# adolfogonzalez3/maddpg

Measured on AMD Instinct MI355X. Metric: env-steps/sec (end-to-end at the reference update cadence), simple_spread N=3, batch 1024, higher is better.
Workload: dtype fp32

## Files before the change

maddpg_amd/csrc/mdp_api.cpp:

```cpp
#include <hip/hip_runtime.h>

#include <algorithm>
#include <cmath>
#include <cstdio>
#include <cstdlib>
#include <cstring>
#include <string>
#include <dlfcn.h>
#include <rccl/rccl.h>

#include <map>
#include <vector>

#include "mdp_kernels.h"

namespace {

inline int64_t r4(int64_t n) { return (n + 3) & ~int64_t(3); }
inline int64_t a256(int64_t n) { return (n + 255) & ~int64_t(255); }

NDesc make_net(int64_t& off, int in, int H, int out) {
  NDesc d;
  d.off = (int)off;
  d.in = in;
// ... 247 lines not shown
  *pos = 624;
}

}

struct mdp_handle {
  mdp_config cfg;
  Layout L;
  int device = 0;
  hipStream_t stream = nullptr;
  bool own_stream = false;
  char* arena = nullptr;
  float *theta, *target, *m, *v, *grad, *replay, *beta, *slab_c, *slab_a, *eplog;
  float *pos, *vel, *ep_rew;
  float* env_comm = nullptr;
  int32_t *index, *goal, *ep_step;
  double *stats, *stat_c, *stat_a, *y;
  Ctl* ctl;
  int64_t len = 0, next = 0;
  uint32_t act_ctr = 0, reset_ctr = 0;
  bool env_lockstep = true;
  std::string err;
  bool ready = false;
  bool prof_on[MDP_K_COUNT] = {};
  std::vector<hipEvent_t> ev[MDP_K_COUNT];
  size_t ev_used[MDP_K_COUNT] = {};
  double prof_ms[MDP_K_COUNT] = {};
  int64_t prof_n[MDP_K_COUNT] = {};
  bool graphs = true;
  bool capturing = false;
  int eager_rounds = 0;
  bool general_grads = false;
  bool fused_apply = true;
  uint32_t* ra_ctr = nullptr;
  uint64_t* ra_part = nullptr;
  float* apre = nullptr;
  bool actor_pre = true;
  float* cpre = nullptr;
  bool critic_pre = true;
  float* apre_rows = nullptr;
  float* cpre_rows = nullptr;
  std::map<std::vector<int>, hipGraphExec_t> graph_exec;
  int eager_steps = 0;
  ncclComm_t comm = nullptr;
  int dp_world = 1;
  bool dp_graphs = false;
  int update_mode = 0;
  FusedApplyArgs* tp_list = nullptr;
  RaBatch tp_batch;
  RaBatch tp_reduce, tp_step;
  int ra_cap = 0, ra_batch_cap = 0;
  bool tp_fits[4] = {true, true, true, true};
  std::vector<FusedApplyArgs> tp_host[4];
  RaBatch tp_xchg;
  RaBatch tp_pair[3][MDP_MAX_AGENTS];
  bool tp_pair_fits[3][MDP_MAX_AGENTS] = {};
  FusedApplyArgs tp_pair_host[3][MDP_MAX_AGENTS][2];
  bool rollout_draw = true;
  bool draw_ahead = true;
  bool grad_pair = true;
  uint64_t* xbuf = nullptr;
  int x_world = 0, x_rank = 0;
  std::vector<void*> x_opened;
  XchgDesc* xd_dev = nullptr;
  uint32_t* x_probe = nullptr;
  uint32_t x_probe_ep = 0;
// ... 680 lines not shown
  if (h->x_probe) (void)hipFree(h->x_probe);
  if (h->xbuf) (void)hipFree(h->xbuf);
  h->xd_dev = nullptr;
  h->x_probe = nullptr;
  h->xbuf = nullptr;
  h->p2p = false;
  h->x_world = 0;
  h->x_rank = 0;
}

int launch_reduce(mdp_handle* h, const OptNet& o) {
  const ReduceArgs a = reduce_args(h, o);
  ProfScope p(h, MDP_K_REDUCE);
  HIPCHK(h, mdp_launch_reduce(a, h->stream));
  return 0;
}

int launch_apply(mdp_handle* h, const OptNet& o, float scale) {
  const ApplyArgs a = apply_args(h, o, scale);
  ProfScope p(h, MDP_K_APPLY);
  HIPCHK(h, mdp_launch_apply(a, h->stream));
  return 0;
}

int opt_step(mdp_handle* h, const OptNet& o, bool fused, float scale, int32_t* pf_out = nullptr, int pf_count = 0) {
  if (fused) {
    FusedApplyArgs f = fused_args(h, o, scale);
    if (pf_out && pf_count > 0) {
      f.pf_out = pf_out;
      f.pf_count = pf_count;
    }
    if (h->p2p && o.own) set_xchg(h, f);
    ProfScope p(h, MDP_K_REDUCE_APPLY);
    HIPCHK(h, mdp_launch_reduce_apply(f, h->stream));
    return 0;
  }
  const int rc = launch_reduce(h, o);
  if (rc) return rc;
  OptNet a = o;
  if (!o.own) a.bump_ctr = 0;
  return launch_apply(h, a, scale);
}

struct RcclApi {
  bool tried = false, ok = false;
  decltype(&ncclGetUniqueId) get_id = nullptr;
  decltype(&ncclCommInitRank) init_rank = nullptr;
  decltype(&ncclAllReduce) all_reduce = nullptr;
  decltype(&ncclCommDestroy) destroy = nullptr;
  decltype(&ncclGetErrorString) err = nullptr;
  decltype(&ncclCommCount) count = nullptr;
};
RcclApi& rccl() {
  static RcclApi r;
  if (!r.tried) {
    r.tried = true;
    const char* alt = getenv("MDP_RCCL_LIB");
    void* so = nullptr;
    if (alt && alt[0]) {
      so = dlopen(alt, RTLD_NOW | RTLD_LOCAL);
    } else {
      so = dlopen("librccl.so.1", RTLD_NOW | RTLD_LOCAL);
      if (!so) so = dlopen("/opt/rocm/lib/librccl.so.1", RTLD_NOW | RTLD_LOCAL);
    }
    if (so) {
      r.get_id = (decltype(r.get_id))dlsym(so, "ncclGetUniqueId");
      r.init_rank = (decltype(r.init_rank))dlsym(so, "ncclCommInitRank");
// ... 167 lines not shown

bool tp_ok(const mdp_handle* h) {
  if (!h->fused_apply) return false;
  for (int i = 0; i < h->cfg.n_agents; ++i)
    if (!reduce_apply_ok(h, i, 0) || !reduce_apply_ok(h, i, 1)) return false;
  return 2 * h->cfg.n_agents <= MDP_RA_BATCH_MAX;
}

FusedApplyArgs tp_args(mdp_handle* h, int agent, int net) {
  const int64_t nwg = h->L.nwg;
  OptNet o = opt_own(h, agent, net);
  o.slab += agent * nwg * o.slab_stride;
  o.slab_stat += agent * nwg * 8;
  o.y += (int64_t)agent * h->cfg.batch_size;
  o.polyak = 1;
  o.bump_ctr = (net == 0 && agent == 0) ? h->cfg.n_agents : 0;
  FusedApplyArgs f = fused_args(h, o);
  for (int t = 0; t < 7; ++t) f.ap.oblk[t] = 0;
  return f;
}

int tp_setup(mdp_handle* h) {
  if (h->tp_list) {
    (void)hipFree(h->tp_list);
    h->tp_list = nullptr;
  }
  const int n = h->cfg.n_agents;
  std::vector<FusedApplyArgs> list;
  RaBatch* rbs[4] = {&h->tp_batch, &h->tp_reduce, &h->tp_step, &h->tp_xchg};
  for (int ph = 0; ph < 4; ++ph) {
    RaBatch& rb = *rbs[ph];
    rb.count = 2 * n;
    rb.narrow = h->L.nwg <= 64 ? 1 : 0;
    rb.wg_start[0] = 0;
    for (int i = 0; i < n; ++i)
      for (int net = 1; net >= 0; --net) {
        FusedApplyArgs f = tp_args(h, i, net);
        f.phase = ph;
        if (ph == 2) f.ap.scale = 1.0f / (float)h->dp_world;
        if (ph == 3) {
          if (h->p2p) set_xchg(h, f);
          else f.phase = 0;
        }
        list.push_back(f);
        const int q = 2 * i + (1 - net);
        rb.wg_start[q + 1] = rb.wg_start[q] + mdp_ra_grid(f);
      }
  }
  for (int ph = 0; ph < 4; ++ph) {
    h->tp_host[ph].assign(list.begin() + 2 * n * ph, list.begin() + 2 * n * (ph + 1));
    h->tp_fits[ph] = ph == 1 || rbs[ph]->wg_start[2 * n] <= h->ra_batch_cap;
  }
  const int pair_phase[3] = {0, 1, 3};
  const size_t pair0 = list.size();
  for (int pp = 0; pp < 3; ++pp)
    for (int i = 0; i < n; ++i) {
      RaBatch& rb = h->tp_pair[pp][i];
      rb = RaBatch();
      rb.count = 2;
      rb.narrow = h->L.nwg <= 64 ? 1 : 0;
      for (int k = 0; k < 2; ++k) {
        const int net = 1 - k;
        FusedApplyArgs f = tp_args(h, i, net);
        f.ap.slab = net ? h->slab_c : h->slab_a;
        f.ap.polyak = 0;
        f.ap.bump_ctr = (net == 0 && i == n - 1) ? n : 0;
        f.phase = pair_phase[pp];
        if (pp == 2) {
          if (h->p2p) set_xchg(h, f);
          else f.phase = 0;
        }
        list.push_back(f);
        h->tp_pair_host[pp][i][k] = f;
        rb.wg_start[k + 1] = rb.wg_start[k] + mdp_ra_grid(f);
      }
      h->tp_pair_fits[pp][i] = pp == 1 || rb.wg_start[2] + 1 <= h->ra_batch_cap;
    }
  HIPCHK(h, hipMalloc((void**)&h->tp_list, sizeof(FusedApplyArgs) * list.size()));
  HIPCHK(h, hipMemcpy(h->tp_list, list.data(), sizeof(FusedApplyArgs) * list.size(), hipMemcpyHostToDevice));
  for (int ph = 0; ph < 4; ++ph) rbs[ph]->list = h->tp_list + (int64_t)ph * 2 * n;
  for (int pp = 0; pp < 3; ++pp)
    for (int i = 0; i < n; ++i) h->tp_pair[pp][i].list = h->tp_list + pair0 + (int64_t)(pp * n + i) * 2;
  return 0;
}

int dp_allreduce_all(mdp_handle* h);
int launch_tp_batch(mdp_handle* h, int ph);

int tp_grads_fast(mdp_handle* h, const int32_t* idx, const float* u_tgt, const float* u_act, int32_t* pf_out) {
  const int n = h->cfg.n_agents;
  const int64_t nwg = h->L.nwg;
  int lds_c = 0;
  for (int i = 0; i < n; ++i) lds_c = std::max(lds_c, lds_critic_r_bytes(h->L.topo, i));
  {
    CriticArgs a;
    a.apre = nullptr;
    a.apre_rows = nullptr;
    a.u_act = nullptr;
    a.cpre = nullptr;
    a.cpre_rows = nullptr;
    a.cpre_prev = -1;
    a.pf_ctl = h->ctl;
    a.pf_out = pf_out;
    a.pf_count = pf_out ? n * h->cfg.batch_size : 0;
    a.topo = h->L.topo;
    a.agent = 0;
    a.B = h->cfg.batch_size;
    a.theta = h->theta;
// ... 38 lines not shown
    a.slab = h->slab_a;
    a.slab_stride = h->L.slab_a;
    a.slab_stat = h->stat_a;
    a.multi = n;
    a.slab_agent_stride = nwg * h->L.slab_a;
    ProfScope p(h, MDP_K_ACTOR_GRAD);
    HIPCHK(h, mdp_launch_actor_grad_r(a, lds_actor_r_bytes(h->L.topo), h->stream));
  }
  return 0;
}

int launch_tp_pair(mdp_handle* h, int pp, int i, int32_t* piece) {
  const int B = h->cfg.batch_size;
  const int kind = pp == 1 ? MDP_K_REDUCE : MDP_K_REDUCE_APPLY;
  if (h->tp_pair_fits[pp][i]) {
    RaBatch rb = h->tp_pair[pp][i];
    if (piece) {
      rb.pf_out = piece;
      rb.pf_count = B;
      rb.pf_ctl = h->ctl;
    }
    ProfScope p(h, kind);
    HIPCHK(h, mdp_launch_reduce_apply_batch(rb, h->stream));
    return 0;
  }
  for (int k = 0; k < 2; ++k) {
    FusedApplyArgs f = h->tp_pair_host[pp][i][k];
    if (piece) {
      f.pf_out = piece + (k ? (B + 1) / 2 : 0);
      f.pf_count = k ? B - (B + 1) / 2 : (B + 1) / 2;
      f.pf_ctl = h->ctl;
    }
    ProfScope p(h, kind);
    HIPCHK(h, mdp_launch_reduce_apply(f, h->stream));
  }
  return 0;
}

int tp_round_general(mdp_handle* h, const int32_t* idx, const float* u_tgt, const float* u_act, int32_t* draw_out) {
  const int n = h->cfg.n_agents;
  const int64_t B = h->cfg.batch_size;
  const int pp = h->comm ? 1 : h->p2p ? 2 : 0;
  int rc;
  for (int i = 0; i < n; ++i) {
    const int32_t* ix = idx + i * B;
    const float* ut = u_tgt ? u_tgt + i * n * B * MDP_ACT_DIM : nullptr;
    const float* ua = u_act ? u_act + i * B * MDP_ACT_DIM : nullptr;
    if (h->grad_pair) {
      GradPairArgs g;
      g.c = critic_args(h, i, ix, ut, true, -1, nullptr, true);
      g.x = actor_args(h, i, ix, ua, true, false, -1, nullptr, true);
      const int lds = std::max(lds_critic_bytes(h->L.topo, g.c.group), lds_actor_bytes(h->L.topo));
      if (lds > MDP_LDS_BUDGET) return fail(h, "gradient pair does not fit in LDS");
      ProfScope p(h, MDP_K_CRITIC_GRAD);
      HIPCHK(h, mdp_launch_grad_pair(g, h->L.topo.H, lds, h->stream));
    } else {
      if ((rc = do_critic_grad(h, i, ix, ut, nullptr, true, false, nullptr, -1, 0, true))) return rc;
      if ((rc = do_actor_grad(h, i, ix, ua, true, false, -1, nullptr, true))) return rc;
    }
    if ((rc = launch_tp_pair(h, pp, i, draw_out ? draw_out + i * B : nullptr))) return rc;
  }
  if (h->comm) {
    if ((rc = dp_allreduce_all(h))) return rc;
    ProfScope p(h, MDP_K_APPLY, h->tp_fits[2]);
    return launch_tp_batch(h, 2);
  }
  float pa, pb;
  polyak_coef(h, &pa, &pb);
  HIPCHK(h, mdp_launch_polyak(h->target, h->theta, h->L.PT, pa, pb, h->ctl, h->stream));
  return 0;
}

int launch_tp_batch(mdp_handle* h, int ph) {
  const RaBatch* rbs[4] = {&h->tp_batch, &h->tp_reduce, &h->tp_step, &h->tp_xchg};
  if (h->tp_fits[ph]) {
    HIPCHK(h, mdp_launch_reduce_apply_batch(*rbs[ph], h->stream));
    return 0;
  }
  for (const FusedApplyArgs& f : h->tp_host[ph]) HIPCHK(h, mdp_launch_reduce_apply(f, h->stream));
  return 0;
}

int do_round_tp(mdp_handle* h, const int32_t* idx, const float* u_tgt, const float* u_act, int32_t* pf_out,
                int32_t* draw_out = nullptr) {
  if (!tp_fast(h)) return tp_round_general(h, idx, u_tgt, u_act, draw_out ? draw_out : pf_out);
  const int rc = tp_grads_fast(h, idx, u_tgt, u_act, pf_out);
  if (rc) return rc;
  if (h->p2p) {
    ProfScope p(h, MDP_K_REDUCE_APPLY, h->tp_fits[3]);
    return launch_tp_batch(h, 3);
  }
  if (h->comm) {
    {
      ProfScope p(h, MDP_K_REDUCE, h->tp_fits[1]);
      const int rc = launch_tp_batch(h, 1);
      if (rc) return rc;
    }
    const int rc = dp_allreduce_all(h);
    if (rc) return rc;
    ProfScope p(h, MDP_K_APPLY, h->tp_fits[2]);
    return launch_tp_batch(h, 2);
  }
  ProfScope p(h, MDP_K_REDUCE_APPLY, h->tp_fits[0]);
  return launch_tp_batch(h, 0);
}

int set_ring(mdp_handle* h, int64_t len, int64_t next) {
  h->len = len;
  h->next = next;
  HIPCHK(h, mdp_launch_set_ring(h->ctl, len, next, h->stream));
  return 0;
}
// ... 205 lines not shown
}

int mdp_ra_plan(const mdp_config* cfg, int32_t cus, int32_t per_cu, int32_t* out) {
  Layout L;
  std::string err;
  if (!build_layout(cfg, L, err) || cus < 0 || per_cu < 0) return -1;
  int fallback = 0;
  for (int i = 0; i < cfg->n_agents; ++i)
    for (int net = 0; net < 2; ++net) {
      const int g = mdp_ra_grid_of(L.topo, i, net);
      const bool ok = mdp_ra_fits(L.topo, i, net, cus * per_cu);
      if (out) out[2 * i + net] = ok ? g : -g;
      fallback += ok ? 0 : 1;
    }
  return fallback;
}

int mdp_create(const mdp_config* cfg, void* arena_dev, int64_t arena_bytes, void* hip_stream, mdp_handle** out) {
  if (!out) return -1;
  *out = nullptr;
  mdp_handle* h = new mdp_handle();
  std::string err;
  if (!build_layout(cfg, h->L, err)) {
    h->err = err;
    *out = h;
    return -1;
  }
  h->cfg = *cfg;
  {
    const char* g = getenv("MDP_GENERAL_GRADS");
    h->general_grads = g && g[0] == '1';
    const char* u = getenv("MDP_UNFUSED_APPLY");
    h->fused_apply = !(u && u[0] == '1');
    const char* rd = getenv("MDP_ROLLOUT_DRAW");
    h->rollout_draw = !(rd && rd[0] == '0');
    const char* da = getenv("MDP_DRAW_AHEAD");
    h->draw_ahead = !(da && da[0] == '0');
    const char* gp = getenv("MDP_GRAD_PAIR");
    h->grad_pair = !(gp && gp[0] == '0');
    const char* ap = getenv("MDP_ACTOR_PRE");
    h->actor_pre = !(ap && ap[0] == '0');
    const char* cp = getenv("MDP_CRITIC_PRE");
    h->critic_pre = !(cp && cp[0] == '0');
  }
  if (!arena_dev || arena_bytes < h->L.total) {
    h->err = "arena missing or too small";
    *out = h;
    return -1;
  }
  *out = h;
  HIPCHK(h, hipGetDevice(&h->device));
  if (need_dev(h, arena_dev, h->L.total, "mdp_create", "arena_dev", false)) return -1;
  {
    int cus = 0, per = 0, per_b = 0;
    HIPCHK(h, hipDeviceGetAttribute(&cus, hipDeviceAttributeMultiprocessorCount, h->device));
    HIPCHK(h, mdp_ra_occupancy(&per));
    HIPCHK(h, mdp_ra_batch_occupancy(&per_b));
    h->ra_cap = cus * per;
    h->ra_batch_cap = cus * per_b;
    int scratch = 0;
    HIPCHK(h, mdp_spin_kernels_scratch(&scratch));
    if (scratch > 0) h->ra_cap = h->ra_batch_cap = 0;
  }
  if (hip_stream) {
    h->stream = (hipStream_t)hip_stream;
  } else {
// ... 1905 lines not shown
```

maddpg_amd/csrc/mdp_apply_fused.hip:

```cpp
#include "mdp_device.h"
#include "mdp_kernels.h"
#include "mdp_mt.h"

namespace {
typedef double f64x4 __attribute__((ext_vector_type(4)));
constexpr uint32_t kSpinLimit = 1u << 22;

__device__ __forceinline__ void st_agent(double* p, double v) {
  __hip_atomic_store(p, v, __ATOMIC_RELAXED, __HIP_MEMORY_SCOPE_AGENT);
}
__device__ __forceinline__ double ld_agent(const double* p) {
  return __hip_atomic_load(const_cast<double*>(p), __ATOMIC_RELAXED, __HIP_MEMORY_SCOPE_AGENT);
}
__device__ __forceinline__ void st_agent64(uint64_t* p, uint64_t v) {
  __hip_atomic_store(p, v, __ATOMIC_RELAXED, __HIP_MEMORY_SCOPE_AGENT);
}
__device__ __forceinline__ uint64_t ld_agent64(const uint64_t* p) {
  return __hip_atomic_load(const_cast<uint64_t*>(p), __ATOMIC_RELAXED, __HIP_MEMORY_SCOPE_AGENT);
}

constexpr uint64_t kXchgTimeoutTicks = 30ull * 100000000ull;

__device__ __forceinline__ uint64_t ll_word(float v, uint32_t ep) {
  return ((uint64_t)ep << 32) | (uint64_t)__float_as_uint(v);
// ... 97 lines not shown
  hipLaunchKernelGGL(k_xchg_probe, dim3(nchunk), dim3(64), 0, s, xd, ep, bad, fault);
  return hipGetLastError();
}

#ifdef MDP_STAMPS
__device__ unsigned long long g_ra_ph[2][1024][8];
#define MDP_RA_PH(k)                                                                                     \
  do {                                                                                                   \
    if (threadIdx.x == 0 && b < 1024) g_ra_ph[a.stats_mode == 1 ? 0 : 1][b][k] = __builtin_amdgcn_s_memrealtime(); \
  } while (0)
extern "C" int mdp_debug_ra_phases(unsigned long long* out) {
  return hipMemcpyFromSymbol(out, HIP_SYMBOL(g_ra_ph), sizeof(g_ra_ph)) == hipSuccess ? 0 : -1;
}
extern "C" int mdp_debug_ra_phases_reset() {
  void* p = nullptr;
  if (hipGetSymbolAddress(&p, HIP_SYMBOL(g_ra_ph)) != hipSuccess) return -1;
  return hipMemset(p, 0, sizeof(unsigned long long) * 2 * 1024 * 8) == hipSuccess && hipDeviceSynchronize() == hipSuccess
             ? 0 : -1;
}
#else
#define MDP_RA_PH(k) \
  do {               \
  } while (0)
#endif

template <int LO, int N>
__device__ __forceinline__ f32x4 red_tree(const f32x4 (*red)[64], int col) {
  if constexpr (N == 1)
    return red[LO][col];
  else
    return red_tree<LO, N / 2>(red, col) + red_tree<LO + N / 2, N / 2>(red, col);
}

template <int G>
__device__ __forceinline__ void reduce_apply_body(const FusedApplyArgs& f, const int b, const uint32_t nb) {
  const ApplyArgs& a = f.ap;
  __shared__ f32x4 red[G][64];
  __shared__ f32x4 gl[64];
  __shared__ float step_l[4];
  const int tid = threadIdx.x, lane = tid & 63;
  MDP_STAMP(30);
  MDP_RA_PH(0);
  if (f.phase == 1 && b >= f.rblk[6]) return;
  if (b < f.rblk[6]) {
    int t = 0;
    while (b >= f.rblk[t + 1]) ++t;
    const TDesc td = a.net.t[t];
    const int n = td.rows * td.cols;
    const int nch = f.rblk[t + 1] - f.rblk[t];
    const int c = b - f.rblk[t];
    const int col = tid & 63, grp = tid >> 6;
    const int p0 = c * MDP_RA_CHUNK + 4 * col;
    const bool act = p0 < n;
    const int64_t i0 = td.off + p0;
    const int pq = c * MDP_RA_CHUNK + 64 * grp + lane;
    const bool aact = grp < 4 && pq < n;
    const int64_t iq = td.off + pq;
    float m1 = 0.f, v1 = 0.f, th1 = 0.f, tg1 = 0.f;
    const float b1p = a.beta[0], b2p = a.beta[1];
    const uint32_t ep_raw = f.phase == 3 ? f.xstep[0] : 0u;
    const uint32_t nep = f.sync_ctr[7 * 32] + 1u;
    uint32_t fault0 = 0u;
    if (grp == 0) fault0 = __hip_atomic_load(&a.ctl->fault, __ATOMIC_RELAXED, __HIP_MEMORY_SCOPE_AGENT);
    bool faulted = false;
    if (aact && f.phase != 1) {
      m1 = a.m[iq];
      v1 = a.v[iq];
      th1 = a.theta[iq];
      if (a.polyak) tg1 = a.target[iq];
    }
    f32x4 s = {0.f, 0.f, 0.f, 0.f};
    if constexpr (G == 16) {
      if (f.phase == 2) {
        if (grp == 0 && act) s = ld4(a.grad + i0);
      } else if (act) {
        const float* base = a.slab + (td.off - a.net.off) + p0;
        f32x4 v[16];
// ... 229 lines not shown
    const uint32_t prev = __hip_atomic_fetch_add(f.done_ctr, 1u, __ATOMIC_RELAXED, __HIP_MEMORY_SCOPE_AGENT);
    if (prev % nb == nb - 1) {
      if (__hip_atomic_load(&a.ctl->fault, __ATOMIC_RELAXED, __HIP_MEMORY_SCOPE_AGENT) == 0u) {
        const float p1 = a.beta[0], p2 = a.beta[1];
        a.beta[2] = p1;
        a.beta[3] = p2;
        a.beta[0] = p1 * a.b1;
        a.beta[1] = p2 * a.b2;
      }
      if (a.bump_ctr) a.ctl->upd_ctr += (uint32_t)a.bump_ctr;
      if (f.phase == 3) f.xstep[0] += 1u;
      f.sync_ctr[7 * 32] += 1u;
    }
  }
}

#ifdef MDP_STAMPS
__device__ unsigned long long g_ra_t0[1024], g_ra_t1[1024];
#define MDP_RA_WG(arr)                                                                 \
  do {                                                                                 \
    if (threadIdx.x == 0 && blockIdx.x < 1024) arr[blockIdx.x] = __builtin_amdgcn_s_memrealtime(); \
  } while (0)
extern "C" int mdp_debug_ra_wg(unsigned long long* t0, unsigned long long* t1, int n) {
  if (hipMemcpyFromSymbol(t0, HIP_SYMBOL(g_ra_t0), sizeof(unsigned long long) * n) != hipSuccess) return -1;
  return hipMemcpyFromSymbol(t1, HIP_SYMBOL(g_ra_t1), sizeof(unsigned long long) * n) == hipSuccess ? 0 : -1;
}
#else
#define MDP_RA_WG(arr) \
  do {                 \
  } while (0)
#endif


template <int NT>
__global__ __launch_bounds__(NT) void k_reduce_apply(FusedApplyArgs f) {
  MDP_RA_WG(g_ra_t0);
  MDP_TL(f.ap.ctl, f.ap.polyak ? 3 : 1, blockIdx.x == gridDim.x - 1 && f.pf_count > 0 ? 3 : 0);
  MDP_KARG_TOUCH("s"(f.pf_count), "s"(f.xstep), "s"(f.ap.blk[0]), "s"(f.ap.target), "s"(f.ap.clip), "s"(f.ap.stats_mode),
                 "s"(f.ap.ctl), "s"(gridDim.x), "s"(f.ap.net.t[0].off), "s"(f.ap.net.t[4].cols), "s"(f.ap.other.t[2].off),
                 "s"(f.ap.other.in));
  if (f.pf_count > 0 && blockIdx.x == gridDim.x - 1) {
    make_index_block<NT>(f.pf_ctl, f.pf_count, f.pf_out);
    __syncthreads();
    MDP_RA_WG(g_ra_t1);
    return;
  }
  reduce_apply_body<NT / 64>(f, blockIdx.x, gridDim.x - (f.pf_count > 0 ? 1 : 0));
#ifdef MDP_STAMPS
  __syncthreads();
  MDP_RA_WG(g_ra_t1);
#endif
}

template <int NT>
__global__ __launch_bounds__(NT) void k_reduce_apply_batch(RaBatch rb) {
  if (rb.pf_count > 0 && blockIdx.x == gridDim.x - 1) {
    make_index_block<NT>(rb.pf_ctl, rb.pf_count, rb.pf_out);
    return;
  }
  int q = 0;
  while (q + 1 < rb.count && (int)blockIdx.x >= rb.wg_start[q + 1]) ++q;
  const int b = blockIdx.x - rb.wg_start[q];
  reduce_apply_body<NT / 64>(rb.list[q], b, (uint32_t)(rb.wg_start[q + 1] - rb.wg_start[q]));
}

int mdp_ra_grid(const FusedApplyArgs& f) {
  const ApplyArgs& a = f.ap;
  return f.rblk[6] + (a.polyak ? a.oblk[6] : 0) + (a.stats_mode ? 1 : 0);
}

#ifndef MDP_RA_NARROW
#define MDP_RA_NARROW 1
#endif
static bool mdp_ra_narrow(const FusedApplyArgs& f) { return MDP_RA_NARROW && f.ap.nwg <= 64; }

hipError_t mdp_launch_reduce_apply(const FusedApplyArgs& f, hipStream_t s) {
  const dim3 grid(mdp_ra_grid(f) + (f.pf_count > 0 ? 1 : 0));
  if (mdp_ra_narrow(f))
    mdp_launch(k_reduce_apply<256>, grid, dim3(256), 0, s, f);
  else
    mdp_launch(k_reduce_apply<1024>, grid, dim3(1024), 0, s, f);
  return hipGetLastError();
}

hipError_t mdp_spin_kernels_scratch(int* bytes) {
  const void* ks[] = {(const void*)k_reduce_apply<256>, (const void*)k_reduce_apply<1024>,
                      (const void*)k_reduce_apply_batch<256>, (const void*)k_reduce_apply_batch<1024>,
                      (const void*)k_xchg_probe};
  *bytes = 0;
  for (const void* k : ks) {
    hipFuncAttributes at;
    const hipError_t e = hipFuncGetAttributes(&at, k);
    if (e != hipSuccess) return e;
    if ((int)at.localSizeBytes > *bytes) *bytes = (int)at.localSizeBytes;
  }
  return hipSuccess;
}

hipError_t mdp_ra_occupancy(int* per_cu) {
  return hipOccupancyMaxActiveBlocksPerMultiprocessor(per_cu, k_reduce_apply<1024>, 1024, 0);
}

hipError_t mdp_ra_batch_occupancy(int* per_cu) {
  return hipOccupancyMaxActiveBlocksPerMultiprocessor(per_cu, k_reduce_apply_batch<1024>, 1024, 0);
}

hipError_t mdp_launch_reduce_apply_batch(const RaBatch& b, hipStream_t s) {
  const dim3 grid(b.wg_start[b.count] + (b.pf_count > 0 ? 1 : 0));
  if (MDP_RA_NARROW && b.narrow)
    mdp_launch(k_reduce_apply_batch<256>, grid, dim3(256), 0, s, b);
  else
    mdp_launch(k_reduce_apply_batch<1024>, grid, dim3(1024), 0, s, b);
  return hipGetLastError();
}

#ifdef MDP_TIMELINE
extern "C" int mdp_debug_tl_ra(unsigned long long* out, int reset) {
  const size_t n = sizeof(unsigned long long) * MDP_TL_SLOTS * MDP_TL_WG * 2;
  if (reset) {
    void* p = nullptr;
    if (hipGetSymbolAddress(&p, HIP_SYMBOL(g_mdp_tl)) != hipSuccess) return -1;
    return hipMemset(p, 0, n) == hipSuccess && hipDeviceSynchronize() == hipSuccess ? 0 : -1;
  }
  return hipMemcpyFromSymbol(out, HIP_SYMBOL(g_mdp_tl), n) == hipSuccess ? 0 : -1;
}
#endif

#ifdef MDP_STAMPS
extern "C" int mdp_debug_stamps_ra(unsigned long long* out, int n) {
  return hipMemcpyFromSymbol(out, HIP_SYMBOL(g_mdp_stamps), sizeof(unsigned long long) * n) == hipSuccess ? 0 : -1;
}
#endif
```

maddpg_amd/csrc/mdp_kernels.h:

```cpp
#pragma once
#include <hip/hip_runtime.h>
#include <hip/hip_ext.h>
#include <stdint.h>

#include <type_traits>

#include "mdp_carve.h"
#include "mdp_topo.h"

struct CriticArgs {
  int agent, B;
  const float* theta;
  const float* target;
  const float* replay;
  const int32_t* idx;
  const float* u_tgt;
  uint64_t seed;
  const Ctl* ctl;
  double gamma;
  float inv_b;
  float* slab;
  int slab_stride;
  double* slab_stat;
  double* y_out;
// ... 93 lines not shown
  float* beta;
  float b1, b2;
  Ctl* ctl;
  int bump_ctr;
};

#define MDP_APPLY_CHUNK 1024

struct ApplyArgs {
  int blk[7], oblk[7];
  float* theta;
  float* target;
  float* m;
  float* v;
  float* grad;
  const float* slab;
  int slab_stride, nwg;
  float scale, clip, lr, b1, b2, eps;
  float* beta;
  int polyak;
  float pa, pb;
  int stats_mode;
  const double* slab_stat;
  const double* y;
  int B;
  float reg;
  double* stats_out;
  uint32_t* ticket;
  Ctl* ctl;
  int bump_ctr;
  NDesc net, other;
};

#define MDP_RA_CHUNK 256
#define MDP_RA_MAXCH 256
#define MDP_XCH_MAXW 8
#define MDP_XCH_PROBE 2048
struct XchgDesc {
  int world, rank;
  int64_t pt;
  uint64_t* data[MDP_XCH_MAXW];
};
inline int64_t mdp_xch_bytes(int world, int64_t param_floats) {
  return 8 * (2 * (int64_t)world * (param_floats + MDP_XCH_PROBE));
}

struct FusedApplyArgs {
  int pf_count;
  int phase;
  int rblk[7];
  uint32_t* sync_ctr;
  uint64_t* sync_part;
  uint32_t* done_ctr;
  const XchgDesc* xd;
  int net_id;
  uint32_t* xstep;
  uint64_t* wstat;
  int32_t* pf_out;
  Ctl* pf_ctl;
  ApplyArgs ap;
};
inline int64_t mdp_ra_sync_bytes() {
  return (int64_t)MDP_MAX_AGENTS * 2 * 8 * 128 + (int64_t)MDP_MAX_AGENTS * 2 * 6 * MDP_RA_MAXCH * 16;
}

#define MDP_PER_STREAM 0x50000u
// ... 280 lines not shown
    (void)hipGetLastError();
    done = true;
  }
}
template <auto K, int LIMIT = MDP_LDS_BUDGET, typename A>
inline hipError_t mdp_launch_lds(const dim3& grid, const dim3& block, int lds, hipStream_t s, const A& a) {
  mdp_raise_lds_limit<K, LIMIT>();
  mdp_launch(K, grid, block, lds, s, a);
  return hipGetLastError();
}

hipError_t mdp_launch_critic_grad(const CriticArgs& a, int H, int lds_bytes, hipStream_t s);
hipError_t mdp_launch_actor_grad(const ActorArgs& a, int H, int lds_bytes, hipStream_t s);
hipError_t mdp_launch_grad_pair(const GradPairArgs& a, int H, int lds_bytes, hipStream_t s);
hipError_t mdp_launch_critic_grad_r(const CriticArgs& a, int lds_bytes, hipStream_t s);
hipError_t mdp_launch_critic_grad_per(const CriticArgsPer& a, int H, int lds_bytes, hipStream_t s);
hipError_t mdp_launch_critic_grad_twin(const CriticArgsTwin& a, int H, int lds_bytes, hipStream_t s);
hipError_t mdp_launch_critic_grad_mm(const CriticArgsMm& a, int H, int lds_bytes, hipStream_t s);
hipError_t mdp_launch_actor_grad_mm(const ActorArgsMm& a, int H, int lds_bytes, hipStream_t s);
hipError_t mdp_launch_critic_grad_apx(const CriticArgsApx& a, int H, int lds_bytes, hipStream_t s);
hipError_t mdp_launch_approx_grad(const ApproxArgs& a, int H, int lds_bytes, hipStream_t s);
hipError_t mdp_launch_critic_grad_r_per(const CriticArgsPer& a, int lds_bytes, hipStream_t s);
hipError_t mdp_launch_actor_grad_r(const ActorArgs& a, int lds_bytes, hipStream_t s);
hipError_t mdp_launch_rollout(const RolloutArgs& a, int H, int lds_bytes, hipStream_t s);
hipError_t mdp_launch_eval(const EvalArgs& a, int H, int lds_bytes, hipStream_t s);
hipError_t mdp_launch_eval_episodes(const EvalEpArgs& a, int H, int lds_bytes, hipStream_t s);
hipError_t mdp_launch_eval_matchups(const EvalMuArgs& a, int H, int lds_bytes, hipStream_t s);
hipError_t mdp_launch_eval_q(const EvalQArgs& a, int H, int lds_bytes, hipStream_t s);
hipError_t mdp_launch_eval_returns(const EvalRetArgs& a, hipStream_t s);
hipError_t mdp_launch_eval_reset(const EnvDesc& env, uint64_t seed, uint32_t first, int count, float* pos, float* vel,
                                 int32_t* goal, hipStream_t s);
hipError_t mdp_launch_apply(const ApplyArgs& a, hipStream_t s);
hipError_t mdp_launch_reduce(const ReduceArgs& a, hipStream_t s);
hipError_t mdp_launch_reduce_apply(const FusedApplyArgs& f, hipStream_t s);
#define MDP_RA_BATCH_MAX (2 * MDP_MAX_AGENTS)
struct RaBatch {
  const FusedApplyArgs* list = nullptr;
  int count = 0;
  int narrow = 0;
  int wg_start[MDP_RA_BATCH_MAX + 1] = {};
  int pf_count = 0;
  int32_t* pf_out = nullptr;
  Ctl* pf_ctl = nullptr;
};
int mdp_ra_grid(const FusedApplyArgs& f);
hipError_t mdp_ra_occupancy(int* per_cu);
hipError_t mdp_spin_kernels_scratch(int* bytes);
inline int mdp_ra_grid_of(const Topo& t, int agent, int net) {
  const NDesc& d = net ? t.ag[agent].critic : t.ag[agent].actor;
  const NDesc& o = net ? t.ag[agent].actor : t.ag[agent].critic;
  int g = 2;
  for (int k = 0; k < 6; ++k) {
    g += (d.t[k].rows * d.t[k].cols + MDP_RA_CHUNK - 1) / MDP_RA_CHUNK;
    if (!net) g += (o.t[k].rows * o.t[k].cols + MDP_APPLY_CHUNK - 1) / MDP_APPLY_CHUNK;
  }
  return g;
}
inline bool mdp_ra_fits(const Topo& t, int agent, int net, int capacity) {
  const NDesc& d = net ? t.ag[agent].critic : t.ag[agent].actor;
  for (int k = 0; k < 6; ++k)
    if ((d.t[k].rows * d.t[k].cols + MDP_RA_CHUNK - 1) / MDP_RA_CHUNK > MDP_RA_MAXCH) return false;
  return mdp_ra_grid_of(t, agent, net) <= capacity;
}
hipError_t mdp_launch_reduce_apply_batch(const RaBatch& b, hipStream_t s);
hipError_t mdp_ra_batch_occupancy(int* per_cu);
hipError_t mdp_launch_xchg_probe(const XchgDesc* xd, uint32_t ep, int nchunk, uint32_t* bad, uint32_t* fault,
                                 hipStream_t s);
// ... 14 lines not shown
```

maddpg_amd/csrc/mdp_kernels.hip:

```cpp
#include <type_traits>

#include "mdp_device.h"
#include "mdp_kernels.h"
#include "mdp_mt.h"

__global__ __launch_bounds__(1024) void k_make_index(Ctl* ctl, int count, int32_t* __restrict__ out) {
  make_index_block<1024>(ctl, count, out);
}

__device__ __forceinline__ void st_nt4(float* o, float4 v) {
  __builtin_nontemporal_store(v.x, o);
  __builtin_nontemporal_store(v.y, o + 1);
  __builtin_nontemporal_store(v.z, o + 2);
  __builtin_nontemporal_store(v.w, o + 3);
}

__global__ __launch_bounds__(256) void k_gather_rows(const float* __restrict__ replay, int stride,
                                                     const int32_t* __restrict__ idx, int count,
                                                     float* __restrict__ out) {
  const uint32_t v4 = (uint32_t)stride >> 2;
  const uint32_t total = (uint32_t)count * v4;
  const uint32_t step = gridDim.x * blockDim.x;
  uint32_t e = blockIdx.x * blockDim.x + threadIdx.x;
  for (; e + 3u * step < total; e += 4u * step) {
// ... 133 lines not shown
    for (int i = 0; i < 4; ++i) h2[(kq * 4 + i) * ldh + col] = fmaxf(acc[i] + b2[t], 0.f);
  }
  __syncthreads();
  if (wave == 0) head_acc<H / 4>(w3, b3, h2, ldh, nd.out, out, ldo);
  __syncthreads();
}

template <int H>
__device__ inline void mlp_fwd_tile(const float* X, int ldx, int K, const float* P, const NDesc& nd, float* h1,
                                    float* h2, int ldh, float* out, int ldo) {
  tile_fwd<true>(X, ldx, K, P + nd.t[0].off, P + nd.t[1].off, H, h1, ldh);
  __syncthreads();
  tile_fwd<true>(h1, ldh, H, P + nd.t[2].off, P + nd.t[3].off, H, h2, ldh);
  __syncthreads();
  if (threadIdx.x < 64) head_mfma<H / 4>(h2, ldh, H, P + nd.t[4].off, P + nd.t[5].off, nd.out, out, ldo);
  __syncthreads();
}

}

namespace {
__device__ inline bool last_block(uint32_t* ticket) {
  int last = 0;
  __syncthreads();
  if (threadIdx.x == 0) {
    __threadfence();
    const uint32_t old = atomicAdd(ticket, 1u);
    last = (old == gridDim.x - 1) ? 1 : 0;
  }
  return __syncthreads_or(last) != 0;
}
}

__global__ __launch_bounds__(256) void k_reduce(ReduceArgs a) {
  const int64_t e = blockIdx.x * (int64_t)blockDim.x + threadIdx.x;
  if (e == 0 && a.beta) {
    const float p1 = a.beta[0], p2 = a.beta[1];
    a.beta[2] = p1;
    a.beta[3] = p2;
    a.beta[0] = p1 * a.b1;
    a.beta[1] = p2 * a.b2;
    if (a.bump_ctr) a.ctl->upd_ctr += 1u;
  }
  const int64_t el = e >> 3;
  const int q = (int)(e & 7);
  float s = 0.f;
  if (el < a.size) {
    const float* p = a.slab + el;
    float v[8], t[24];
#pragma unroll
    for (int k = 0; k < 8; ++k) {
      const int w = q + 8 * k;
      v[k] = w < a.nwg ? p[(int64_t)w * a.slab_stride] : 0.f;
    }
#pragma unroll
    for (int k = 0; k < 24; ++k) {
      const int w = q + 64 + 8 * k;
      t[k] = w < a.nwg ? p[(int64_t)w * a.slab_stride] : 0.f;
    }
#pragma unroll
    for (int k = 0; k < 24; ++k)
      if (q + 64 + 8 * k < a.nwg) s += t[k];
    for (int w = q + 256; w < a.nwg; w += 8) s += p[(int64_t)w * a.slab_stride];
#pragma unroll
    for (int k = 0; k < 8; ++k) s += v[k];
  }
  s = half_row_sum(s);
  if (el < a.size && q == 0) a.grad[a.off + el] = s;
}

__global__ __launch_bounds__(256) void k_apply(ApplyArgs a) {
  __shared__ double red[4];
  const int b = blockIdx.x;
  const int tid = threadIdx.x;
  const float b1p = a.beta[2], b2p = a.beta[3];
  if (b < a.blk[6]) {
    int t = 0;
    while (b >= a.blk[t + 1]) ++t;
    const TDesc td = a.net.t[t];
    const int n = td.rows * td.cols;
    const float* g = a.grad + td.off;
    constexpr int PT = MDP_APPLY_CHUNK / 256;
    const int e0 = (b - a.blk[t]) * MDP_APPLY_CHUNK;
    const int e1 = min(n, e0 + MDP_APPLY_CHUNK);
    float cg[PT], cm[PT], cv[PT], cth[PT], ctg[PT];
#pragma unroll
    for (int q = 0; q < PT; ++q) {
      const int e = min(e0 + tid + q * 256, e1 - 1);
      const int64_t i = td.off + e;
      cg[q] = g[e];
      cm[q] = a.m[i];
      cv[q] = a.v[i];
      cth[q] = a.theta[i];
      ctg[q] = a.polyak ? a.target[i] : 0.f;
    }
    double ss = 0.0;
    for (int f0 = tid; f0 < n; f0 += 8 * blockDim.x) {
      float v[8];
#pragma unroll
      for (int q = 0; q < 8; ++q) {
// ... 1054 lines not shown
  return mdp_for_width(H, [&](auto h) {
    return launch_env<k_eval_episodes<h.value>>(dim3(row_tiles(a.episodes)), lds_bytes, s, a);
  });
}
hipError_t mdp_launch_eval_matchups(const EvalMuArgs& a, int H, int lds_bytes, hipStream_t s) {
  return mdp_for_width(H, [&](auto h) {
    return launch_env<k_eval_episodes<h.value, EvalMuArgs>>(dim3(row_tiles(a.episodes), a.matchups), lds_bytes, s, a);
  });
}
hipError_t mdp_launch_eval_q(const EvalQArgs& a, int H, int lds_bytes, hipStream_t s) {
  return mdp_for_width(H, [&](auto h) {
    return launch_env<k_eval_episodes<h.value, EvalQArgs>>(dim3(row_tiles(a.episodes)), lds_bytes, s, a);
  });
}
hipError_t mdp_launch_eval_returns(const EvalRetArgs& a, hipStream_t s) {
  const int64_t total = (int64_t)a.episodes * a.n;
  mdp_launch(k_eval_returns, dim3((unsigned)((total + 255) / 256)), dim3(256), 0, s, a);
  MDP_CHECK_LAUNCH();
  return hipSuccess;
}
hipError_t mdp_launch_eval_reset(const EnvDesc& env, uint64_t seed, uint32_t first, int count, float* pos, float* vel,
                                 int32_t* goal, hipStream_t s) {
  hipLaunchKernelGGL(k_eval_reset, dim3((count + 255) / 256), dim3(256), 0, s, env, seed, first, count, pos, vel, goal);
  MDP_CHECK_LAUNCH();
  return hipSuccess;
}
hipError_t mdp_launch_apply(const ApplyArgs& a, hipStream_t s) {
  const int grid = a.blk[6] + (a.polyak ? a.oblk[6] : 0) + (a.stats_mode ? 1 : 0);
  mdp_launch(k_apply, dim3(grid), dim3(256), 0, s, a);
  MDP_CHECK_LAUNCH();
  return hipSuccess;
}
hipError_t mdp_launch_reduce(const ReduceArgs& a, hipStream_t s) {
  const int grid = (int)((a.size * 8 + 255) / 256);
  mdp_launch(k_reduce, dim3(grid), dim3(256), 0, s, a);
  MDP_CHECK_LAUNCH();
  return hipSuccess;
}
hipError_t mdp_launch_make_index(Ctl* ctl, int count, int32_t* out, hipStream_t s) {
  mdp_launch(k_make_index, dim3(1), dim3(1024), 0, s, ctl, count, out);
  MDP_CHECK_LAUNCH();
  return hipSuccess;
}
__global__ __launch_bounds__(256) void k_polyak(float* __restrict__ target, const float* __restrict__ theta,
                                                int64_t n4, float pa, float pb, const Ctl* ctl) {
  if (__hip_atomic_load(&ctl->fault, __ATOMIC_RELAXED, __HIP_MEMORY_SCOPE_AGENT) != 0u) return;
  for (int64_t i = (int64_t)blockIdx.x * 256 + threadIdx.x; i < n4; i += (int64_t)gridDim.x * 256) {
    const f32x4 tg = reinterpret_cast<const f32x4*>(target)[i];
    const f32x4 th = reinterpret_cast<const f32x4*>(theta)[i];
    f32x4 o;
#pragma unroll
    for (int j = 0; j < 4; ++j) o[j] = pa * tg[j] + pb * th[j];
    reinterpret_cast<f32x4*>(target)[i] = o;
  }
}
hipError_t mdp_launch_polyak(float* target, const float* theta, int64_t n, float pa, float pb, const Ctl* ctl,
                             hipStream_t s) {
  const int64_t n4 = n / 4;
  const int grid = (int)std::min<int64_t>(1024, (n4 + 255) / 256);
  mdp_launch(k_polyak, dim3(grid > 0 ? grid : 1), dim3(256), 0, s, target, theta, n4, pa, pb, ctl);
  MDP_CHECK_LAUNCH();
  return hipSuccess;
}
hipError_t mdp_launch_gather(const float* replay, int stride, const int32_t* idx, int count, float* out,
                             hipStream_t s) {
  const int v4 = stride >> 2;
  const int per = (int)((((int64_t)1 << 31) - 1) / v4);
  for (int b0 = 0; b0 < count; b0 += per) {
// ... 79 lines not shown
```

Before: 1.122 million.

## Add lane-parallel register path for fused gradient reduce and Adam apply

Adds a new reduce_apply_lanes body for narrow (nwg<=64) phase-0 fused reduce+apply launches. Each 16-lane row sums a float4 column slice across workgroup partials, and cross-row sums use permlane swaps instead of shared-memory trees. The path is selected via a new LANES template and a narrow==2 batch flag, with an MDP_RA_LANES env switch that defaults to on. The unfused k_reduce is also rewritten to use 4 or 16 lanes per element to match the fused layout. The aim is to cut shared-memory traffic and barrier cost in the small-network optimizer step, at the cost of more template variants and a changed summation order.

```diff
diff --git a/maddpg_amd/csrc/mdp_api.cpp b/maddpg_amd/csrc/mdp_api.cpp
--- a/maddpg_amd/csrc/mdp_api.cpp
+++ b/maddpg_amd/csrc/mdp_api.cpp
@@ -303,6 +303,7 @@
   int eager_rounds = 0;
   bool general_grads = false;
   bool fused_apply = true;
+  bool ra_lanes = true;
   uint32_t* ra_ctr = nullptr;
   uint64_t* ra_part = nullptr;
   float* apre = nullptr;
@@ -1049,7 +1050,7 @@
     }
     if (h->p2p && o.own) set_xchg(h, f);
     ProfScope p(h, MDP_K_REDUCE_APPLY);
-    HIPCHK(h, mdp_launch_reduce_apply(f, h->stream));
+    HIPCHK(h, mdp_launch_reduce_apply(f, h->stream, h->ra_lanes));
     return 0;
   }
   const int rc = launch_reduce(h, o);
@@ -1283,6 +1284,7 @@
     RaBatch& rb = *rbs[ph];
     rb.count = 2 * n;
     rb.narrow = h->L.nwg <= 64 ? 1 : 0;
+    bool lanes = h->ra_lanes && ph == 0;
     rb.wg_start[0] = 0;
     for (int i = 0; i < n; ++i)
       for (int net = 1; net >= 0; --net) {
@@ -1294,9 +1296,11 @@
           else f.phase = 0;
         }
         list.push_back(f);
+        lanes = lanes && mdp_ra_lanes(f);
         const int q = 2 * i + (1 - net);
         rb.wg_start[q + 1] = rb.wg_start[q] + mdp_ra_grid(f);
       }
+    if (lanes) rb.narrow = 2;
   }
   for (int ph = 0; ph < 4; ++ph) {
     h->tp_host[ph].assign(list.begin() + 2 * n * ph, list.begin() + 2 * n * (ph + 1));
@@ -1310,6 +1314,7 @@
       rb = RaBatch();
       rb.count = 2;
       rb.narrow = h->L.nwg <= 64 ? 1 : 0;
+      bool lanes = h->ra_lanes && pp == 0;
       for (int k = 0; k < 2; ++k) {
         const int net = 1 - k;
         FusedApplyArgs f = tp_args(h, i, net);
@@ -1323,8 +1328,10 @@
         }
         list.push_back(f);
         h->tp_pair_host[pp][i][k] = f;
+        lanes = lanes && mdp_ra_lanes(f);
         rb.wg_start[k + 1] = rb.wg_start[k] + mdp_ra_grid(f);
       }
+      if (lanes) rb.narrow = 2;
       h->tp_pair_fits[pp][i] = pp == 1 || rb.wg_start[2] + 1 <= h->ra_batch_cap;
     }
   HIPCHK(h, hipMalloc((void**)&h->tp_list, sizeof(FusedApplyArgs) * list.size()));
@@ -1429,7 +1436,7 @@
       f.pf_ctl = h->ctl;
     }
     ProfScope p(h, kind);
-    HIPCHK(h, mdp_launch_reduce_apply(f, h->stream));
+    HIPCHK(h, mdp_launch_reduce_apply(f, h->stream, h->ra_lanes));
   }
   return 0;
 }
@@ -1474,7 +1481,7 @@
     HIPCHK(h, mdp_launch_reduce_apply_batch(*rbs[ph], h->stream));
     return 0;
   }
-  for (const FusedApplyArgs& f : h->tp_host[ph]) HIPCHK(h, mdp_launch_reduce_apply(f, h->stream));
+  for (const FusedApplyArgs& f : h->tp_host[ph]) HIPCHK(h, mdp_launch_reduce_apply(f, h->stream, h->ra_lanes));
   return 0;
 }
 
@@ -1746,6 +1753,8 @@
     h->general_grads = g && g[0] == '1';
     const char* u = getenv("MDP_UNFUSED_APPLY");
     h->fused_apply = !(u && u[0] == '1');
+    const char* rl = getenv("MDP_RA_LANES");
+    h->ra_lanes = !(rl && rl[0] == '0');
     const char* rd = getenv("MDP_ROLLOUT_DRAW");
     h->rollout_draw = !(rd && rd[0] == '0');
     const char* da = getenv("MDP_DRAW_AHEAD");
diff --git a/maddpg_amd/csrc/mdp_apply_fused.hip b/maddpg_amd/csrc/mdp_apply_fused.hip
--- a/maddpg_amd/csrc/mdp_apply_fused.hip
+++ b/maddpg_amd/csrc/mdp_apply_fused.hip
@@ -153,8 +153,150 @@
     return red_tree<LO, N / 2>(red, col) + red_tree<LO + N / 2, N / 2>(red, col);
 }
 
-template <int G>
+__device__ __forceinline__ double row_sum_d(double v) {
+  v += dpp_d<0xB1, 0xf>(v);
+  v += dpp_d<0x4E, 0xf>(v);
+  v += dpp_d<0x141, 0xf>(v);
+  v += dpp_d<0x140, 0xf>(v);
+  return v;
+}
+
+__device__ __forceinline__ float rows_sum(float v) {
+#if __has_builtin(__builtin_amdgcn_permlane16_swap) && __has_builtin(__builtin_amdgcn_permlane32_swap)
+  const auto p = __builtin_amdgcn_permlane16_swap(__float_as_uint(v), __float_as_uint(v), false, false);
+  v = __uint_as_float(p[0]) + __uint_as_float(p[1]);
+  const auto h = __builtin_amdgcn_permlane32_swap(__float_as_uint(v), __float_as_uint(v), false, false);
+  return __uint_as_float(h[0]) + __uint_as_float(h[1]);
+#else
+  const float o = __shfl_xor(v, 16, 64);
+  v = (threadIdx.x & 16) ? o + v : v + o;
+  const float u = __shfl_xor(v, 32, 64);
+  return (threadIdx.x & 32) ? u + v : v + u;
+#endif
+}
+
+__device__ __forceinline__ double chunks_poll(const uint64_t* part, int nch, uint32_t nep, int lane, uint32_t* fault,
+                                              bool* faulted) {
+  double tot = 0.0;
+  for (int q = lane; q < nch; q += 64) {
+    uint64_t hi = ld_agent64(part + 2 * q), lo = ld_agent64(part + 2 * q + 1);
+    uint32_t it = 0;
+    while ((uint32_t)(hi >> 32) != nep || (uint32_t)(lo >> 32) != nep) {
+      __builtin_amdgcn_s_sleep(1);
+      if (++it > kSpinLimit) {
+        __hip_atomic_store(fault, 1u, __ATOMIC_RELAXED, __HIP_MEMORY_SCOPE_AGENT);
+        *faulted = true;
+        break;
+      }
+      hi = ld_agent64(part + 2 * q);
+      lo = ld_agent64(part + 2 * q + 1);
+    }
+    tot += __longlong_as_double((long long)((hi << 32) | (lo & 0xffffffffull)));
+  }
+  return wave_sum_d(tot);
+}
+
+__device__ __forceinline__ void reduce_apply_lanes(const FusedApplyArgs& f, const int b) {
+  const ApplyArgs& a = f.ap;
+  const int lane = threadIdx.x & 63;
+  const int wq = __builtin_amdgcn_readfirstlane((int)(threadIdx.x >> 6));
+  const int g = lane >> 4;
+  int t = 0;
+  while (b >= f.rblk[t + 1]) ++t;
+  const TDesc td = a.net.t[t];
+  const int n = td.rows * td.cols;
+  const int nch = f.rblk[t + 1] - f.rblk[t];
+  const int c = b - f.rblk[t];
+  const int q0 = c * MDP_RA_CHUNK + 64 * wq;
+  const bool wact = q0 < n;
+  const int p0 = q0 + 4 * (lane & 15);
+  const bool act = p0 < n;
+  const int pq = p0 + g;
+  const bool aact = pq < n;
+  const int64_t iq = td.off + pq;
+  float m1 = 0.f, v1 = 0.f, th1 = 0.f, tg1 = 0.f;
+  const float b1p = a.beta[0], b2p = a.beta[1];
+  const uint32_t nep = f.sync_ctr[7 * 32] + 1u;
+  const uint32_t fault0 = __hip_atomic_load(&a.ctl->fault, __ATOMIC_RELAXED, __HIP_MEMORY_SCOPE_AGENT);
+  if (aact) {
+    m1 = a.m[iq];
+    v1 = a.v[iq];
+    th1 = a.theta[iq];
+    if (a.polyak) tg1 = a.target[iq];
+  }
+  f32x4 s = {0.f, 0.f, 0.f, 0.f};
+  if (act) {
+    const float* base = a.slab + (td.off - a.net.off) + p0;
+    f32x4 v[16];
+#pragma unroll
+    for (int k = 0; k < 16; ++k) v[k] = ld4(base + (int64_t)min(g + 4 * k, a.nwg - 1) * a.slab_stride);
+#pragma unroll
+    for (int k = 0; k < 16; ++k)
+      if (g + 4 * k >= a.nwg) v[k] = f32x4{0.f, 0.f, 0.f, 0.f};
+    s = ((v[0] + v[1]) + v[2]) + v[3];
+#pragma unroll
+    for (int k = 4; k < 16; ++k)
+      if (g + 4 * k < a.nwg) s += v[k];
+  }
+#pragma unroll
+  for (int j = 0; j < 4; ++j) s[j] = rows_sum(s[j]);
+#ifdef MDP_STAMPS
+  asm volatile("" ::"v"(s[0]), "v"(s[3]));
+#endif
+  MDP_RA_PH(1);
+  double ss = 0.0;
+#pragma unroll
+  for (int j = 0; j < 4; ++j) {
+    const float gs = s[j] * a.scale;
+    if (p0 + j < n) ss += (double)gs * (double)gs;
+  }
+  ss = row_sum_d(ss);
+  __shared__ double sq_l[4];
+  asm volatile("s_waitcnt vmcnt(0) lgkmcnt(0)" ::: "memory");
+  if (lane == 0) sq_l[wq] = ss;
+  __syncthreads();
+  ss = (sq_l[3] + sq_l[2]) + (sq_l[1] + sq_l[0]);
+  MDP_RA_PH(2);
+  uint64_t* part = f.sync_part + (int64_t)t * MDP_RA_MAXCH * 2;
+  if (nch > 1 && threadIdx.x == 0) {
+    const uint64_t tag = (uint64_t)nep << 32;
+    const uint64_t bits = (uint64_t)__double_as_longlong(ss);
+    st_agent64(part + 2 * c, tag | (bits >> 32));
+    st_agent64(part + 2 * c + 1, tag | (bits & 0xffffffffull));
+  }
+  const float gq = g == 0 ? s[0] : g == 1 ? s[1] : g == 2 ? s[2] : s[3];
+  if (aact) a.grad[iq] = gq;
+  if (a.stats_mode && threadIdx.x == 0)
+    __hip_atomic_fetch_add(f.done_ctr, 1u, __ATOMIC_RELAXED, __HIP_MEMORY_SCOPE_AGENT);
+  MDP_RA_PH(3);
+  double tot = ss;
+  bool faulted = false;
+  if (wact) {
+    if (nch > 1) tot = chunks_poll(part, nch, nep, lane, &a.ctl->fault, &faulted);
+    faulted = __ballot(faulted || ctr_use(fault0) != 0u) != 0ull;
+  }
+  const float norm = (float)sqrt(tot);
+  MDP_RA_PH(4);
+  if (aact && !faulted) {
+    const float clip = a.clip;
+    const float denom = fmaxf(norm, clip);
+    const float one = 1.0f;
+    const float alpha = a.lr * sqrtf(one - b2p) / (one - b1p);
+    const float c1 = one - a.b1, c2 = one - a.b2;
+    const float gc = ((gq * a.scale) * clip) / denom;
+    const float mo = m1 + (gc - m1) * c1;
+    const float vo = v1 + (gc * gc - v1) * c2;
+    const float tho = th1 - (mo * alpha) / (sqrtf(vo) + a.eps);
+    a.m[iq] = mo;
+    a.v[iq] = vo;
+    a.theta[iq] = tho;
+    if (a.polyak) a.target[iq] = a.pa * tg1 + a.pb * tho;
+  }
+}
+
+template <int G, bool LANES = false>
 __device__ __forceinline__ void reduce_apply_body(const FusedApplyArgs& f, const int b, const uint32_t nb) {
+  static_assert(!LANES || G == 4, "the register body is a narrow launch");
   const ApplyArgs& a = f.ap;
   __shared__ f32x4 red[G][64];
   __shared__ f32x4 gl[64];
@@ -163,7 +305,9 @@
   MDP_STAMP(30);
   MDP_RA_PH(0);
   if (f.phase == 1 && b >= f.rblk[6]) return;
-  if (b < f.rblk[6]) {
+  if (LANES && b < f.rblk[6]) {
+    reduce_apply_lanes(f, b);
+  } else if (b < f.rblk[6]) {
     int t = 0;
     while (b >= f.rblk[t + 1]) ++t;
     const TDesc td = a.net.t[t];
@@ -459,7 +603,7 @@
 #endif
 
 
-template <int NT>
+template <int NT, bool LANES = false>
 __global__ __launch_bounds__(NT) void k_reduce_apply(FusedApplyArgs f) {
   MDP_RA_WG(g_ra_t0);
   MDP_TL(f.ap.ctl, f.ap.polyak ? 3 : 1, blockIdx.x == gridDim.x - 1 && f.pf_count > 0 ? 3 : 0);
@@ -472,14 +616,14 @@
     MDP_RA_WG(g_ra_t1);
     return;
   }
-  reduce_apply_body<NT / 64>(f, blockIdx.x, gridDim.x - (f.pf_count > 0 ? 1 : 0));
+  reduce_apply_body<NT / 64, LANES>(f, blockIdx.x, gridDim.x - (f.pf_count > 0 ? 1 : 0));
 #ifdef MDP_STAMPS
   __syncthreads();
   MDP_RA_WG(g_ra_t1);
 #endif
 }
 
-template <int NT>
+template <int NT, bool LANES = false>
 __global__ __launch_bounds__(NT) void k_reduce_apply_batch(RaBatch rb) {
   if (rb.pf_count > 0 && blockIdx.x == gridDim.x - 1) {
     make_index_block<NT>(rb.pf_ctl, rb.pf_count, rb.pf_out);
@@ -488,7 +632,7 @@
   int q = 0;
   while (q + 1 < rb.count && (int)blockIdx.x >= rb.wg_start[q + 1]) ++q;
   const int b = blockIdx.x - rb.wg_start[q];
-  reduce_apply_body<NT / 64>(rb.list[q], b, (uint32_t)(rb.wg_start[q + 1] - rb.wg_start[q]));
+  reduce_apply_body<NT / 64, LANES>(rb.list[q], b, (uint32_t)(rb.wg_start[q + 1] - rb.wg_start[q]));
 }
 
 int mdp_ra_grid(const FusedApplyArgs& f) {
@@ -496,14 +640,15 @@
   return f.rblk[6] + (a.polyak ? a.oblk[6] : 0) + (a.stats_mode ? 1 : 0);
 }
 
-#ifndef MDP_RA_NARROW
-#define MDP_RA_NARROW 1
-#endif
 static bool mdp_ra_narrow(const FusedApplyArgs& f) { return MDP_RA_NARROW && f.ap.nwg <= 64; }
 
-hipError_t mdp_launch_reduce_apply(const FusedApplyArgs& f, hipStream_t s) {
+bool mdp_ra_lanes(const FusedApplyArgs& f) { return mdp_ra_narrow(f) && f.phase == 0; }
+
+hipError_t mdp_launch_reduce_apply(const FusedApplyArgs& f, hipStream_t s, bool lanes) {
   const dim3 grid(mdp_ra_grid(f) + (f.pf_count > 0 ? 1 : 0));
-  if (mdp_ra_narrow(f))
+  if (lanes && mdp_ra_lanes(f))
+    mdp_launch(k_reduce_apply<256, true>, grid, dim3(256), 0, s, f);
+  else if (mdp_ra_narrow(f))
     mdp_launch(k_reduce_apply<256>, grid, dim3(256), 0, s, f);
   else
     mdp_launch(k_reduce_apply<1024>, grid, dim3(1024), 0, s, f);
@@ -513,6 +658,7 @@
 hipError_t mdp_spin_kernels_scratch(int* bytes) {
   const void* ks[] = {(const void*)k_reduce_apply<256>, (const void*)k_reduce_apply<1024>,
                       (const void*)k_reduce_apply_batch<256>, (const void*)k_reduce_apply_batch<1024>,
+                      (const void*)k_reduce_apply<256, true>, (const void*)k_reduce_apply_batch<256, true>,
                       (const void*)k_xchg_probe};
   *bytes = 0;
   for (const void* k : ks) {
@@ -534,7 +680,9 @@
 
 hipError_t mdp_launch_reduce_apply_batch(const RaBatch& b, hipStream_t s) {
   const dim3 grid(b.wg_start[b.count] + (b.pf_count > 0 ? 1 : 0));
-  if (MDP_RA_NARROW && b.narrow)
+  if (MDP_RA_NARROW && b.narrow == 2)
+    mdp_launch(k_reduce_apply_batch<256, true>, grid, dim3(256), 0, s, b);
+  else if (MDP_RA_NARROW && b.narrow)
     mdp_launch(k_reduce_apply_batch<256>, grid, dim3(256), 0, s, b);
   else
     mdp_launch(k_reduce_apply_batch<1024>, grid, dim3(1024), 0, s, b);
diff --git a/maddpg_amd/csrc/mdp_kernels.h b/maddpg_amd/csrc/mdp_kernels.h
--- a/maddpg_amd/csrc/mdp_kernels.h
+++ b/maddpg_amd/csrc/mdp_kernels.h
@@ -149,6 +149,9 @@
   NDesc net, other;
 };
 
+#ifndef MDP_RA_NARROW
+#define MDP_RA_NARROW 1
+#endif
 #define MDP_RA_CHUNK 256
 #define MDP_RA_MAXCH 256
 #define MDP_XCH_MAXW 8
@@ -495,7 +498,8 @@
                                  int32_t* goal, hipStream_t s);
 hipError_t mdp_launch_apply(const ApplyArgs& a, hipStream_t s);
 hipError_t mdp_launch_reduce(const ReduceArgs& a, hipStream_t s);
-hipError_t mdp_launch_reduce_apply(const FusedApplyArgs& f, hipStream_t s);
+hipError_t mdp_launch_reduce_apply(const FusedApplyArgs& f, hipStream_t s, bool lanes);
+bool mdp_ra_lanes(const FusedApplyArgs& f);
 #define MDP_RA_BATCH_MAX (2 * MDP_MAX_AGENTS)
 struct RaBatch {
   const FusedApplyArgs* list = nullptr;
diff --git a/maddpg_amd/csrc/mdp_kernels.hip b/maddpg_amd/csrc/mdp_kernels.hip
--- a/maddpg_amd/csrc/mdp_kernels.hip
+++ b/maddpg_amd/csrc/mdp_kernels.hip
@@ -189,7 +189,9 @@
 }
 }
 
+template <int G>
 __global__ __launch_bounds__(256) void k_reduce(ReduceArgs a) {
+  static_assert(G == 4 || G == 16, "the fused launch's 4 or 16 waves");
   const int64_t e = blockIdx.x * (int64_t)blockDim.x + threadIdx.x;
   if (e == 0 && a.beta) {
     const float p1 = a.beta[0], p2 = a.beta[1];
@@ -199,30 +201,24 @@
     a.beta[1] = p2 * a.b2;
     if (a.bump_ctr) a.ctl->upd_ctr += 1u;
   }
-  const int64_t el = e >> 3;
-  const int q = (int)(e & 7);
+  const int64_t el = e / G;
+  const int q = (int)(e & (G - 1));
   float s = 0.f;
   if (el < a.size) {
     const float* p = a.slab + el;
-    float v[8], t[24];
-#pragma unroll
-    for (int k = 0; k < 8; ++k) {
-      const int w = q + 8 * k;
+    float v[16];
+#pragma unroll
+    for (int k = 0; k < 16; ++k) {
+      const int w = q + G * k;
       v[k] = w < a.nwg ? p[(int64_t)w * a.slab_stride] : 0.f;
     }
-#pragma unroll
-    for (int k = 0; k < 24; ++k) {
-      const int w = q + 64 + 8 * k;
-      t[k] = w < a.nwg ? p[(int64_t)w * a.slab_stride] : 0.f;
-    }
-#pragma unroll
-    for (int k = 0; k < 24; ++k)
-      if (q + 64 + 8 * k < a.nwg) s += t[k];
-    for (int w = q + 256; w < a.nwg; w += 8) s += p[(int64_t)w * a.slab_stride];
-#pragma unroll
-    for (int k = 0; k < 8; ++k) s += v[k];
-  }
-  s = half_row_sum(s);
+    s = ((v[0] + v[1]) + v[2]) + v[3];
+#pragma unroll
+    for (int k = 4; k < 16; ++k)
+      if (q + G * k < a.nwg) s += v[k];
+    for (int w = q + 16 * G; w < a.nwg; w += G) s += p[(int64_t)w * a.slab_stride];
+  }
+  s = G == 4 ? quad_sum(s) : row_sum(s);
   if (el < a.size && q == 0) a.grad[a.off + el] = s;
 }
 
@@ -1343,8 +1339,10 @@
   return hipSuccess;
 }
 hipError_t mdp_launch_reduce(const ReduceArgs& a, hipStream_t s) {
-  const int grid = (int)((a.size * 8 + 255) / 256);
-  mdp_launch(k_reduce, dim3(grid), dim3(256), 0, s, a);
+  if (MDP_RA_NARROW && a.nwg <= 64)
+    mdp_launch(k_reduce<4>, dim3((int)((a.size * 4 + 255) / 256)), dim3(256), 0, s, a);
+  else
+    mdp_launch(k_reduce<16>, dim3((int)((a.size * 16 + 255) / 256)), dim3(256), 0, s, a);
   MDP_CHECK_LAUNCH();
   return hipSuccess;
 }
```

Result: faster. 1.141 million, median of 6 (+1.7%).
